# aconley/mbb_emcee

Hardware: AMD Instinct MI355X
Metric: walker-likelihood evals/sec (+ MCMC steps/sec), 250 walkers × 8 bands, 1/2/4/8 GPU (higher is better)
Workload: dtype f64; 1 GPU; cfg2/cfg3: 8 passbands (NQ 2209) with full response integration, thick+alpha, 250 walkers per GPU, device-resident stretch move; 1 step = 2 dependent half-steps; walkers_per_gpu=250, walkers=250, bands=8, nq=2209, sampler_form=form 7: one launch per <=4096 steps, preconditioning=50 ms of scratch-ensemble steps before the W warm-up steps (GPU clocks)

## Files before the change

### include/mbb_hip.h

```cpp
#ifndef MBB_HIP_H
#define MBB_HIP_H

#include <stddef.h>
#include <stdint.h>

#ifdef __cplusplus
extern "C" {
#endif

typedef struct mbb_ctx mbb_ctx;

enum mbb_error {
    MBB_OK = 0,
    MBB_ERR_HIP = -1,
    MBB_ERR_ARG = -2,
    MBB_ERR_STATE = -3,
    MBB_ERR_RCCL = -4
};

enum mbb_row_status {
    MBB_ROW_OK = 0,
    MBB_ROW_BELOW_LOWLIM = 1,
    MBB_ROW_BAD_ALPHA = 2,
    MBB_ROW_BAD_BETA = 3,
// ... 31 lines not shown
                            double *d_lnl, int32_t *d_status, double *d_model_flux);

int mbb_lnlike_repeat_device(mbb_ctx *ctx, const double *d_pars, int n, double *d_lnl,
                             int32_t *d_status, int reps);

int mbb_roof_probe(mbb_ctx *ctx, const double pars[5], int reps, double *seconds,
                   double *lane_slots, double *clock_mhz);

int mbb_sampler_create(mbb_ctx *ctx, int nwalkers, unsigned long long seed, void **sampler);
int mbb_sampler_destroy(mbb_ctx *ctx, void *sampler);
int mbb_sampler_reset(mbb_ctx *ctx, void *sampler);
int mbb_sampler_set_state(mbb_ctx *ctx, void *sampler, const double *pos, const double *lnprob);
int mbb_sampler_run(mbb_ctx *ctx, void *sampler, int nsteps, double stretch_a, double *chain,
                    double *lnprob, double *pos_out, double *lnprob_out, double *naccepted);
int mbb_sampler_advance_async(mbb_ctx *ctx, void *sampler, int nsteps, double stretch_a);
int mbb_sampler_advance_timed(mbb_ctx *ctx, void *sampler, int nsteps, double stretch_a, double *wall_s,
                              float *stream_ms);

#define MBB_SUMMARY_COLS 8
#define MBB_SUMMARY_MAX_PCT 8
enum mbb_summary_derived { MBB_SUM_PEAK = 1, MBB_SUM_LIR = 2, MBB_SUM_DUSTMASS = 4 };
enum mbb_summary_status {
    MBB_SUM_EMPTY = 1,
    MBB_SUM_HAS_NAN = 2,
    MBB_SUM_ABSENT = 4,
    MBB_SUM_ROW_SHIFT = 8
};
typedef struct mbb_summary_spec {
    int32_t npct;
    int32_t burn, thin;
// ... 71 lines not shown
```

### mbb_emcee_amd/_native.py

```python
import ctypes as C
import os

import numpy as np

_HERE = os.path.dirname(os.path.abspath(__file__))
LIB_PATH = os.path.join(_HERE, "libmbb_hip.so")

ROW_OK, ROW_BELOW_LOWLIM, ROW_BAD_ALPHA, ROW_BAD_BETA, ROW_NOCONV, ROW_NONFINITE = 0, 1, 2, 3, 6, 7

_dp = C.POINTER(C.c_double)
_ip = C.POINTER(C.c_int32)
_vp = C.c_void_p

SUMMARY_COLS, SUMMARY_MAX_PCT = 8, 8
SUM_PEAK, SUM_LIR, SUM_DUSTMASS = 1, 2, 4
SUM_EMPTY, SUM_HAS_NAN, SUM_ABSENT, SUM_ROW_SHIFT = 1, 2, 4, 8


class SummarySpec(C.Structure):
    _fields_ = [("npct", C.c_int32), ("burn", C.c_int32), ("thin", C.c_int32), ("derived", C.c_int32),
                ("peak_model", C.c_int32),
                ("has_lo", C.c_int32 * SUMMARY_COLS), ("has_hi", C.c_int32 * SUMMARY_COLS),
                ("pct", C.c_double * SUMMARY_MAX_PCT),
                ("lo", C.c_double * SUMMARY_COLS), ("hi", C.c_double * SUMMARY_COLS),
# ... 23 lines not shown
    "mbb_lnlike_call": (C.c_int, [_vp, C.c_int]),
    "mbb_boundary_generation": (_vp, [_vp]),
    "mbb_lnlike_batch_device": (C.c_int, [_vp, _vp, C.c_int, _vp, _vp, _vp]),
    "mbb_lnlike_repeat_device": (C.c_int, [_vp, _vp, C.c_int, _vp, _vp, C.c_int]),
    "mbb_roof_probe": (C.c_int, [_vp, _dp, C.c_int, _dp, _dp, _dp]),
    "mbb_sampler_create": (C.c_int, [_vp, C.c_int, C.c_ulonglong, C.POINTER(_vp)]),
    "mbb_sampler_destroy": (C.c_int, [_vp, _vp]),
    "mbb_sampler_reset": (C.c_int, [_vp, _vp]),
    "mbb_sampler_set_state": (C.c_int, [_vp, _vp, _dp, _dp]),
    "mbb_sampler_run": (C.c_int, [_vp, _vp, C.c_int, C.c_double, _dp, _dp, _dp, _dp, _dp]),
    "mbb_chain_summary": (C.c_int, [_vp, _dp, _dp, C.c_int, C.c_int, C.c_int, C.POINTER(SummarySpec),
                                    C.POINTER(SummaryOut)]),
    "mbb_sampler_run_summary": (C.c_int, [_vp, _vp, C.c_int, C.c_double, C.POINTER(SummarySpec),
                                          C.POINTER(SummaryOut), _dp, _dp, _dp, _dp, _dp]),
    "mbb_sampler_advance_async": (C.c_int, [_vp, _vp, C.c_int, C.c_double]),
    "mbb_sampler_advance_timed": (C.c_int, [_vp, _vp, C.c_int, C.c_double, C.POINTER(C.c_double), C.POINTER(C.c_float)]),
    "mbb_sed_prologue_batch": (C.c_int, [_vp, _dp, C.c_int, C.c_int, C.c_int, C.c_double,
                                         C.c_int, _dp, _ip]),
    "mbb_sed_eval_batch": (C.c_int, [_vp, _dp, C.c_int, C.c_int, C.c_int, C.c_double, _dp,
                                     C.c_int, _dp, _ip]),
    "mbb_sed_integrate_batch": (C.c_int, [_vp, _dp, C.c_int, C.c_int, C.c_int, C.c_double, C.c_double,
                                          C.c_double, _dp, _ip]),
    "mbb_fnu_eval": (C.c_int, [_vp, C.c_int, C.c_int, _dp, C.c_int] + [C.c_double] * 7 + [_dp]),
    "mbb_malloc": (C.c_int, [_vp, C.c_size_t, C.POINTER(_vp)]),
    "mbb_free": (C.c_int, [_vp, _vp]),
    "mbb_memcpy_h2d": (C.c_int, [_vp, _vp, _vp, C.c_size_t]),
    "mbb_memcpy_d2h": (C.c_int, [_vp, _vp, _vp, C.c_size_t]),
    "mbb_sync": (C.c_int, [_vp]),
    "mbb_stream": (_vp, [_vp]),
    "mbb_event_create": (C.c_int, [_vp, C.POINTER(_vp)]),
# ... 329 lines not shown
```

### mbb_emcee_amd/csrc/mbb_flow_index.h

```cpp
#pragma once
#if defined(__HIPCC__)
#define MBB_FLOW_HD __host__ __device__
#else
#define MBB_FLOW_HD
#endif

constexpr int kFlowSlots = 4;
constexpr int kFlowLag = 4;

MBB_FLOW_HD constexpr int flow_cnt(int h, int j) { return (j - h + 1) > 0 ? (j - h + 1) >> 1 : 0; }
MBB_FLOW_HD constexpr int flow_seq(int h, int m) { return m > 0 ? h + 2 * m - 1 : 0; }

constexpr int kFmSlots = 4;
constexpr int kFmMseq = kFmSlots;
constexpr int kFmLag = 4;
constexpr int kFmRing = 8;
constexpr int kFmNC = 3;
constexpr int kFmNB = 4;
```

### mbb_emcee_amd/csrc/mbb_flowa.hip.h

```cpp
#pragma once
#include "mbb_flowm.hip.h"


template <bool OPTHIN, bool NOALPHA, bool STAGE>
__global__ void __launch_bounds__(1024) k_flowa(const LikeArgs a_val)
{
    CLikeArgs *const ka = MBB_KERNARGS();
    extern __shared__ __align__(16) unsigned char smem_raw[];
    __shared__ __align__(16) double s_tab[kExp2N];
    __shared__ __align__(16) double s_pb[kPolyBDoubles];
    __shared__ __align__(16) double s_pc[OPTHIN ? 2 : kPolyCDoubles];
    const int tid = threadIdx.x, lane = tid & 63, wave = MBB_WAVE_ID(tid);
#define MBB_FA_COMMON() \
    const int W = a.wpb; \
    const int nun = a.nunit, npart = a.npart, nb = a.nb; \
    const int nC = (2 * W + 3) >> 2, nQ = 16 - nC; \
    WalkerK *wk0 = reinterpret_cast<WalkerK *>(smem_raw);                          \
    double *partial0 = reinterpret_cast<double *>(wk0 + kFaNB * W);               \
    double *rec0 = partial0 + kFaNB * (size_t)W * npart;                          \
    double *mflux = rec0 + kFaNB * (size_t)W * kFaRec;                            \
    double *own = mflux + (size_t)W * nb;                                         \
    double *s_flux = own + 2 * (size_t)W * 8; \
    double *s_ivar = s_flux + nb; \
    double *s_invcov = s_ivar + nb; \
    int2 *s_band = reinterpret_cast<int2 *>(s_invcov + (a.cov_in_lds ? (size_t)nb * nb : 0)); \
    int *ctl = reinterpret_cast<int *>(s_band + nb + 1);                          \
    const size_t tab_off = ((size_t)(reinterpret_cast<unsigned char *>(ctl + 48) - smem_raw) + 15) & ~(size_t)15; \
    double *s_nu = reinterpret_cast<double *>(smem_raw + tab_off); \
    double *s_lnnu = s_nu + (STAGE ? a.nchunk * 64 : 0); \
    double *s_wt = s_lnnu + (STAGE ? a.nchunk * 64 : 0); \
    const int wbase = (int)blockIdx.x * W; \
    const int Wl = min(W, a.n - wbase); \
    const FlowMView fv = flowm_view(a.spec, a.nw); \
    const unsigned long long serial32 = a.flow_serial << 32; \
    unsigned long long *const done_set = fv.done + (size_t)(a.spec_cfg & 1) * kFmRing * 16; \
    const long long spin_limit = flow_spin_limit(a.spec_cfg); \
    const int niter = a.persist; \
    int *const c_ready = ctl + 16, *const c_qdone = ctl + 32, *const c_edone = ctl + 4; \
    (void)nun; (void)nQ; (void)mflux; (void)own; (void)s_flux; (void)s_ivar; (void)s_invcov; (void)s_nu; (void)s_lnnu; (void)s_wt; \
    (void)Wl; (void)done_set; (void)spin_limit; (void)niter; (void)c_ready; (void)c_qdone; (void)c_edone; (void)partial0; (void)rec0

    {
        MBB_ROLE_ARGS();
        MBB_FA_COMMON();
        const int nt = (int)blockDim.x;
        if (tid < 48) ctl[tid] = 0;
        if (tid < 2 * W * 6) {
            const int hh = tid / (W * 6), l = (tid - hh * W * 6) / 6, e = tid % 6;
            if (l < Wl) {
                const int r = (hh ? a.c_count : 0) + wbase + l;
                const double v = a.pos6[(size_t)r * 6 + e];
                own[(size_t)(hh * W + l) * 8 + e] = v;
                fm_put(fv.row + (size_t)r * kFmWords + 2 * e, v, serial32);
            }
        }
        if (blockIdx.x == 0 && tid < kFmRing * 16)
            __hip_atomic_store(fv.done + (size_t)((a.spec_cfg & 1) ^ 1) * kFmRing * 16 + tid, 0ull, __ATOMIC_RELAXED, __HIP_MEMORY_SCOPE_AGENT);
        const double2 *gb = reinterpret_cast<const double2 *>(a.poly_b);
        const double2 *gc = reinterpret_cast<const double2 *>(a.poly_c);
        double2 *lb = reinterpret_cast<double2 *>(s_pb);
        double2 *lc = reinterpret_cast<double2 *>(s_pc);
        for (int i = tid; i < kExp2N; i += nt) s_tab[i] = kExp2Tab[i];
        for (int i = tid; i < kPolyBDoubles / 2; i += nt) lb[i] = gb[i];
        if (!OPTHIN)
            for (int i = tid; i < kPolyCDoubles / 2; i += nt) lc[i] = gc[i];
        for (int b = tid; b < nb; b += nt) { s_flux[b] = a.flux[b]; s_ivar[b] = a.ivar[b]; s_band[b] = a.band_rng[b]; }
        if (a.cov_in_lds)
            for (int i = tid; i < nb * nb; i += nt) s_invcov[i] = a.invcov[i];
        if (STAGE) {
            const int n2 = a.nchunk * 32;
            const double2 *g0 = reinterpret_cast<const double2 *>(a.nu), *g1 = reinterpret_cast<const double2 *>(a.lnnu),
                          *g2 = reinterpret_cast<const double2 *>(a.wt);
// ... 206 lines not shown
            const int row = sb + wbase + l;
            const bool c1 = cand && j > 0;
            const bool active = l < Wl && (cand == 0 || j > 0);
            double zz = 1.0, u3 = 0.5;
            int pj = 0;
            if (active) stretch_draw(row, a.step + (j >> 1), h, a.seed + 0x9E3779B97F4A7C15ull * (unsigned long long)(j >> 1),
                                     a.stretch_a, a.c_count, zz, pj, u3);
            const int prow = ob + pj;
            const int m1 = flow_cnt(h ^ 1, j), m0 = flow_cnt(h ^ 1, j - 1);
            if (j >= kFaNB) lds_wait(c_edone + bj, Wl * MBB_FA_TURN(j - kFaNB));
            const double *src = c1 ? fv.prop + (((size_t)prow * kFmSlots + (m1 % kFmSlots)) * 2) * kFmWords + 2 * (l16 < 5 ? l16 : 0)
                                   : fv.row + ((size_t)(m0 % kFmSlots) * a.nw + prow) * kFmWords + 2 * (l16 < 5 ? l16 : 0);
            const unsigned long long tag = serial32 | (unsigned long long)(c1 ? j : flow_seq(h ^ 1, m0));
            const bool want_e = active && l16 < 5, want_g = ci == 0 && lane == 5 && j >= kFmLag;
            const unsigned long long need_g = (unsigned long long)gridDim.x * (unsigned long long)nC * (unsigned long long)(((j - kFmLag) / kFmRing) + 1);
            const unsigned long long *gword = done_set + ((j - kFmLag) & (kFmRing - 1)) * 16;
            if (ci == 0) FA_EV(j, 8);
            double pv = 0.0;
            {
                bool ok = !(want_e || want_g);
                long long spins = 0;
                for (;;) {
                    if (want_e && !ok) ok = fm_get(src, tag, pv);
                    if (want_g && !ok) ok = __hip_atomic_load(gword, __ATOMIC_RELAXED, __HIP_MEMORY_SCOPE_AGENT) >= need_g;
                    if (__builtin_amdgcn_ballot_w64(!ok) == 0) break;
                    ++spins;
                    if (spins > spin_limit ||
                        ((spins & 255) == 8 && __hip_atomic_load(a.errflag, __ATOMIC_RELAXED, __HIP_MEMORY_SCOPE_AGENT) != 0)) {
                        atomicMax(a.errflag, 9);
                        break;
                    }
// ... 53 lines not shown
                    if (now && lane == pbase) __hip_atomic_store(c_ready + bj * 8 + l, MBB_FA_TURN(j), __ATOMIC_RELAXED, __HIP_MEMORY_SCOPE_WORKGROUP);
                    if (__builtin_amdgcn_ballot_w64(!handed) == 0) break;
                    ++spins;
                    if (spins > spin_limit ||
                        ((spins & 255) == 8 && __hip_atomic_load(a.errflag, __ATOMIC_RELAXED, __HIP_MEMORY_SCOPE_AGENT) != 0)) {
                        atomicMax(a.errflag, 9);
                        break;
                    }
                    __builtin_amdgcn_s_sleep(1);
                    if (watch2 && !handed) v2 = __hip_atomic_load(w2, __ATOMIC_RELAXED, __HIP_MEMORY_SCOPE_AGENT);
                }
            }
            if (ci == 0) FA_EV(j, 11);
            MBB_FM_ORDER();
            if (ci == 0) FA_EV(j, 12);
            if (lane == 0) __hip_atomic_fetch_add(done_set + (j & (kFmRing - 1)) * 16, 1ull, __ATOMIC_RELAXED, __HIP_MEMORY_SCOPE_AGENT);
        }
    }
#undef MBB_FA_COMMON
#undef MBB_FA_TURN
#undef FA_EV
}
```

### mbb_emcee_amd/csrc/mbb_flowm.hip.h

```cpp
#pragma once
#include "mbb_kernels.hip.h"

__device__ __forceinline__ long long flow_spin_limit(int spec_cfg)
{
    const int v = (spec_cfg >> 24) & 0x3f;
    return v == 63 ? 0ll : 1ll << (v ? v : 22);
}

constexpr int kFmReady = 0;
constexpr int kFmQDone = 4;
constexpr int kFmEDone = 8;
constexpr int kFmPen = 16;
constexpr int kFmStaged = 12;
constexpr int kFmLooks = 8;
constexpr int kFmPrioChain = 3, kFmPrioCtor = 2, kFmPrioWait = 1;

__device__ __forceinline__ int fm_loop_lane(int l)
{
    asm volatile("" : "+v"(l));
    return l;
}
__device__ __forceinline__ void fm_put(double *pair, double v, unsigned long long tag)
{
    typedef unsigned int u32x4 __attribute__((ext_vector_type(4)));
// ... 40 lines not shown
    double *s_ivar = s_flux + nb; \
    double *s_invcov = s_ivar + nb; \
    int2 *s_band = reinterpret_cast<int2 *>(s_invcov + (a.cov_in_lds ? (size_t)nb * nb : 0)); \
    double *cscr = reinterpret_cast<double *>(s_band + nb + 1); \
    int *ctl0 = reinterpret_cast<int *>(cscr + kFmNC * 64); \
    const size_t unit_off = ((size_t)(reinterpret_cast<unsigned char *>(ctl0 + 32 * NP) - smem_raw) + 15) & ~(size_t)15; \
    int4 *s_unit = reinterpret_cast<int4 *>(smem_raw + unit_off);     \
    int *s_tail = reinterpret_cast<int *>(s_unit + nun);               \
    const size_t tab_off = unit_off + (size_t)kFmUnitBytes * nun; \
    double *s_nu = reinterpret_cast<double *>(smem_raw + tab_off); \
    double *s_lnnu = s_nu + (STAGE ? a.nchunk * 64 : 0); \
    double *s_wt = s_lnnu + (STAGE ? a.nchunk * 64 : 0); \
    const long long spin_limit = flow_spin_limit(a.spec_cfg); \
    const FlowMView fv = flowm_view(a.spec, a.nw); \
    const unsigned long long serial32 = a.flow_serial << 32; \
    unsigned long long *const done_set = fv.done + (size_t)(a.spec_cfg & 1) * kFmRing * 16; \
    const int niter = a.persist;
#define MBB_FM_PAIRS_LOOP _Pragma("clang loop unroll(disable)")
#define MBB_FM_PAIR(vp) \
    const int w = wbase + (vp); \
    if constexpr (NP > 1) { if (w >= a.n) continue; }       \
    WalkerK *const wk = wk0 + (vp) * kFmNB; \
    double *const partial = partial0 + (size_t)(vp) * kFmNB * npart; \
    double *const prop = prop0 + (vp) * kFmNB * kFmProp; \
    int *const ctl = ctl0 + 32 * (vp); \
    (void)wk; (void)partial; (void)prop; (void)ctl
#define MBB_FM_ORDER() do { __builtin_amdgcn_fence(__ATOMIC_ACQ_REL, "wavefront"); __builtin_amdgcn_wave_barrier(); } while (0)
#define MBB_FM_WAITS() \
    auto dec_ok = [&](unsigned long long v, unsigned long long need) {    \
        return (v >> 32) == (serial32 >> 32) && ((v & 0xffffffffull) >> 1) >= need; \
    }; \
// ... 33 lines not shown
    const int tid = threadIdx.x, lane = tid & 63, wave = MBB_WAVE_ID(tid);
    const int nwave = blockDim.x >> 6, nq = nwave - kFmNC - 2;
    const bool spread = nwave == 16;
    const int role = spread ? (wave == 3 ? 1 : wave == 7 ? 2 : wave == 14 ? 3 : wave == 11 ? 1 + kFmNC : wave == 15 ? 2 + kFmNC : 0)
                            : (wave < nq ? 0 : 1 + wave - nq);
    const int qi = spread ? wave - (wave >> 2) : wave;
    {
        MBB_ROLE_ARGS();
        MBB_FM_COMMON();
        if (tid < 32 * NP) ctl0[tid] = 0;
        if (cand == 0 && tid < 12 * NP && wbase + tid / 12 < a.n) {
            const int t12 = tid % 12;
            const int r = (t12 < 6 ? 0 : a.c_count) + wbase + tid / 12, e = t12 < 6 ? t12 : t12 - 6;
            fm_put(fv.row + (size_t)r * kFmWords + 2 * e, a.pos6[(size_t)r * 6 + e], serial32);
        }
        if (blockIdx.x == 0 && tid < kFmRing * 16)
            __hip_atomic_store(fv.done + (size_t)((a.spec_cfg & 1) ^ 1) * kFmRing * 16 + tid, 0ull, __ATOMIC_RELAXED, __HIP_MEMORY_SCOPE_AGENT);
        (void)done_set; (void)niter; (void)spin_limit;
    }
    __syncthreads();
#ifdef MBB_STAMPS
    if (tid == 0 && a.stamps) a.stamps[(1u << 20) + 4096 + blockIdx.x] = __builtin_amdgcn_s_memrealtime();
    unsigned long long t_acc[8] = {0, 0, 0, 0, 0, 0, 0, 0};
    unsigned long long t_last = __builtin_amdgcn_s_memtime();
#define FM_T(kk) do { const unsigned long long t_now = __builtin_amdgcn_s_memtime(); t_acc[kk] += t_now - t_last; t_last = t_now; } while (0)
#define FM_TD(kk, dep) do { asm volatile("" ::"v"(dep)); FM_T(kk); } while (0)
#define FM_TOUT() do { if (lane == 0 && a.stamps) for (int kk = 0; kk < 8; ++kk) a.stamps[((size_t)blockIdx.x * 16 + wave) * 8 + kk] = t_acc[kk]; } while (0)
    if (lane == 0 && a.stamps) {
        unsigned hwid, xcc;
        asm volatile("s_getreg_b32 %0, hwreg(HW_REG_HW_ID)" : "=s"(hwid));
        asm volatile("s_getreg_b32 %0, hwreg(HW_REG_XCC_ID)" : "=s"(xcc));
        a.stamps[(1u << 20) + blockIdx.x * 16 + wave] = ((unsigned long long)xcc << 32) | hwid;
// ... 145 lines not shown
        MBB_FM_PAIRS_LOOP
        for (int vp = 0; vp < NP; ++vp) {
            MBB_FM_PAIR(vp);
            const int b = it & (kFmNB - 1);
            const int L_step = a.step + (it >> 1), L_half = it & 1;
            const unsigned long long L_seed = a.seed + 0x9E3779B97F4A7C15ull * (unsigned long long)(it >> 1);
            const int row = (L_half ? a.c_count : 0) + w, c_begin = L_half ? 0 : a.c_count;
            double zz, u3;
            int pj;
            stretch_draw(row, L_step, L_half, L_seed, a.stretch_a, a.c_count, zz, pj, u3);
            const int prow = c_begin + pj;
            const int m_par = flow_cnt(L_half ^ 1, it), m_s = flow_cnt(L_half, it);
            const unsigned long long need_p = (unsigned long long)flow_seq(L_half ^ 1, m_par);
            const double *lnp_p = fv.row + ((size_t)(m_s % kFmSlots) * a.nw + row) * kFmWords + 10;
            const unsigned long long tag_s = serial32 | (unsigned long long)flow_seq(L_half, m_s);
            const unsigned long long need_g = 2ull * (unsigned long long)a.n * (unsigned long long)(((it - kFmLag) / kFmRing) + 1);
            const unsigned long long *word = lane == 22 ? fv.mseq + (size_t)prow * kFmMseq + (m_par % kFmSlots)
                                                        : done_set + ((it - kFmLag) & (kFmRing - 1)) * 16;
            const bool watch = (lane == 22 && need_p > 0) || (lane == 23 && it >= kFmLag);
            const WalkerK *wkb = wk + b;
            const double *pr = prop + b * kFmProp;
            int st = ROW_SKIP;
            double cbb = 0.0, pen_u = 0.0, pen_g = 0.0, lnz4 = 0.0, lnu = 0.0, acc = 0.0;
            double q[5] = {0.0, 0.0, 0.0, 0.0, 0.0}, old5[5] = {0.0, 0.0, 0.0, 0.0, 0.0};
            bool have_rec = false;
            auto record = [&]() {
                st = wkb->status;
                cbb = wkb->cq; pen_u = pr[7]; pen_g = pr[8];
#pragma unroll
                for (int i = 0; i < 5; ++i) { q[i] = pr[i]; old5[i] = pr[9 + i]; }
                lnz4 = pr[5]; lnu = pr[6];
                have_rec = true;
            };
            auto sums = [&]() {
// ... 40 lines not shown
            };
            const int q_need = nq * ((it / kFmNB) + 1);
            FM_EV(it, 9);
#ifdef MBB_STAMPS
            unsigned long long t_ok = 0;
#endif
            unsigned long long pv = 0;
            double lnp = 0.0;
            bool ok = !(watch || lane == 21), have_sums = false;
            long long spins = 0;
            __builtin_amdgcn_s_setprio(kFmPrioWait);
            for (;;) {
                double lv;
                unsigned long long lchk, wv;
                const bool ask_l = lane == 21 && !ok, ask_w = watch && !ok;
                if (ask_l) {
                    lv = ld_dev(lnp_p);
                    lchk = __hip_atomic_load(reinterpret_cast<const unsigned long long *>(lnp_p) + 1, __ATOMIC_RELAXED, __HIP_MEMORY_SCOPE_AGENT);
                }
                if (ask_w) wv = __hip_atomic_load(word, __ATOMIC_RELAXED, __HIP_MEMORY_SCOPE_AGENT);
#pragma nounroll
                for (int look = 0; !have_sums; ++look) {
                    if (!have_rec && __hip_atomic_load(ctl + kFmPen + b, __ATOMIC_RELAXED, __HIP_MEMORY_SCOPE_WORKGROUP) >= it + 1) {
                        MBB_FM_ORDER();
                        record();
                    }
                    if (__hip_atomic_load(ctl + kFmQDone + b, __ATOMIC_RELAXED, __HIP_MEMORY_SCOPE_WORKGROUP) >= q_need) {
                        MBB_FM_ORDER();
                        FM_EV(it, 4);
                        sums();
                        have_sums = true;
                        break;
                    }
                    if (look >= kFmLooks) break;
                    __builtin_amdgcn_s_sleep(1);
                }
                if (ask_l) asm volatile("" : "+v"(lv), "+v"(lchk));
                if (ask_w) asm volatile("" : "+v"(wv));
                if (ask_l) { lnp = lv; ok = (lchk ^ (unsigned long long)__double_as_longlong(lv)) == tag_s; }
                if (ask_w) { pv = wv; ok = lane == 22 ? dec_ok(pv, need_p) : pv >= need_g; }
#ifdef MBB_STAMPS
                if ((ask_l || ask_w) && ok) t_ok = __builtin_amdgcn_s_memrealtime();
#endif
                if (__builtin_amdgcn_ballot_w64(!ok) == 0) break;
                ++spins;
                if (spins > spin_limit ||
                    ((spins & 255) == 8 && __hip_atomic_load(a.errflag, __ATOMIC_RELAXED, __HIP_MEMORY_SCOPE_AGENT) != 0)) {
                    atomicMax(a.errflag, 9);
                    break;
                }
                __builtin_amdgcn_s_sleep(1);
            }
            __builtin_amdgcn_s_setprio(kFmPrioChain);
            const int flag = (need_p > 0 && (fm_lane_lo<22>(pv) & 1u)) ? 1 : 0;
            const bool mine = flag == cand;
            const double lnp_cur = fm_lane<21>(lnp);
            FM_TD(0, lnp_cur);
            FM_EV(it, 5);
            FM_EVV(it, 7, prow);
#ifdef MBB_STAMPS
            { const unsigned long long t21 = __shfl(t_ok, 21), t22 = __shfl(t_ok, 22), t23 = __shfl(t_ok, 23);
              FM_EVV(it, 10, t21); FM_EVV(it, 11, t22); FM_EVV(it, 12, t23); }
#endif
            if (!have_sums) {
                lds_wait(ctl + kFmQDone + b, q_need);
                FM_T(1);
                FM_EV(it, 4);
                sums();
            }
            FM_TD(2, acc);
            {
                double r;
                if (st == ROW_BELOW_LOWLIM) r = -__builtin_inf();
                else if (st != ROW_OK) r = __builtin_nan("");
                else {
                    r = fma(-0.5, acc, pen_u);
// ... 10 lines not shown
                                           __HIP_MEMORY_SCOPE_AGENT);
                    const double lnp_new = accept ? r : lnp_cur;
                    double ve = lnp_new;
#pragma unroll
                    for (int i = 0; i < 5; ++i) ve = ((lane & 7) == i) ? (accept ? q[i] : old5[i]) : ve;
                    if (lane < 6)
                        fm_put(fv.row + ((size_t)(m_new % kFmSlots) * a.nw + row) * kFmWords + 2 * lane, ve,
                               serial32 | (unsigned long long)(it + 1));
                    __builtin_amdgcn_s_setprio(kFmPrioWait);
                    if (lane < 6) { if (it + 2 >= niter) a.pos6[(size_t)row * 6 + lane] = ve; }
                    else if (lane >= 8 && lane < 14 && a.chain6)
                        a.chain6[((size_t)it * a.n + w) * 6 + (lane - 8)] = ve;
                    if (lane == 0 && accept) atomicAdd(a.nacc + (size_t)L_half * a.n + w, 1u);
                }
                __builtin_amdgcn_s_setprio(kFmPrioWait);
                if (lane == 0) __hip_atomic_fetch_add(done_set + (it & (kFmRing - 1)) * 16, 1ull, __ATOMIC_RELAXED, __HIP_MEMORY_SCOPE_AGENT);
            }
            FM_T(3);
        }
        FM_TOUT();
        return;
    }

    {
        MBB_ROLE_ARGS();
        MBB_FM_COMMON();
        MBB_FM_WAITS();
        MBB_PIN(a.c_count); MBB_PIN(a.step); MBB_PIN(a.seed); MBB_PIN(a.stretch_a); MBB_PIN(a.nw); MBB_PIN(a.errflag); MBB_PIN(a.zpow);
        MBB_PIN(a.lowlim[0]); MBB_PIN(a.lowlim[1]); MBB_PIN(a.lowlim[2]); MBB_PIN(a.lowlim[3]); MBB_PIN(a.lowlim[4]);
        MBB_PIN(a.nunorm); MBB_PIN(a.lnunorm); MBB_PIN(a.has_uplim); MBB_PIN(a.has_gprior);
        const int cb = role - 1;
// ... 197 lines not shown
```

### mbb_emcee_amd/csrc/mbb_hip.hip

```cpp
#include <hip/hip_runtime.h>
#include <dlfcn.h>
#include <math.h>
#include <stdint.h>
#include <stdio.h>
#include <stdlib.h>
#include <string.h>
#include <time.h>

#include <algorithm>
#include <functional>
#include <string>
#include <type_traits>
#include <atomic>
#include <chrono>
#include <mutex>
#include <thread>
#include <vector>

#include "../../include/mbb_hip.h"
#include "mbb_device.hip.h"
#include "mbb_kernels.hip.h"
#include "mbb_summary.hip.h"

#define MBB_FLOW_EXT(OT, NA)                                                    \
// ... 1147 lines not shown
    if (rc) return rc;
    mbb_sampler_state *s = (mbb_sampler_state *)sp;
    if (!s) return MBB_OK;
    HIPCHK(hipStreamSynchronize(c->stream));
    if (s->pos6_owned) free_dev(s->d_pos6);
    else if (c->x.users > 0) --c->x.users;
    free_dev(s->d_nacc); free_dev(s->d_err); free_dev(s->d_chain6); free_dev(s->d_chain_out); free_dev(s->d_spec);
    if (s->h_chain) (void)hipHostFree(s->h_chain);
    free_dev(s->d_bak);
    delete s;
    return MBB_OK;
}

static int sampler_check_pending(mbb_ctx *c, mbb_sampler_state *s);

extern "C" int mbb_sampler_reset(mbb_ctx *c, void *sp)
{
    int rc = use(c);
    if (rc) return rc;
    mbb_sampler_state *s = (mbb_sampler_state *)sp;
    if (!s) return fail(MBB_ERR_ARG, "null sampler");
    (void)sampler_check_pending(c, s);
    HIPCHK(hipStreamSynchronize(c->stream));
    HIPCHK(hipMemset(s->d_nacc, 0, (size_t)s->rows() * sizeof(unsigned int)));
    HIPCHK(hipMemset(s->d_err, 0, sizeof(int)));
    return MBB_OK;
}

extern "C" int mbb_sampler_set_state(mbb_ctx *c, void *sp, const double *pos, const double *lnprob)
{
// ... 271 lines not shown
    if (rp.resting) --c->flow_rest;
    if (rp.form >= 7) {
        const size_t R = (size_t)s->rows();
        if (!s->d_spec) {
            HIPCHK(hipMalloc((void **)&s->d_spec, spec_words(R) * sizeof(double)));
            HIPCHK(hipMemsetAsync(s->d_spec, 0, spec_words(R) * sizeof(double), c->stream));
        }
        if (backup) {
            if (!s->d_bak) HIPCHK(hipMalloc((void **)&s->d_bak, R * 6 * sizeof(double) + R * sizeof(unsigned int)));
            HIPCHK(hipMemcpyAsync(s->d_bak, s->d_pos6, R * 6 * sizeof(double), hipMemcpyDeviceToDevice, c->stream));
            HIPCHK(hipMemcpyAsync(s->d_bak + R * 6, s->d_nacc, R * sizeof(unsigned int), hipMemcpyDeviceToDevice, c->stream));
        }
        s->backup_kept = backup;
        if (s->spec_form != 7 && s->spec_form != 9) {
            const FlowMView fvh = flowm_view(s->d_spec, (int)R);
            HIPCHK(hipMemsetAsync(fvh.done, 0, 2 * kFmRing * 16 * sizeof(unsigned long long), c->stream));
            s->flowm_parity = 0;
        }
        s->spec_form = rp.form;
    }
    const bool carried = tev && rp.form >= 7 && nsteps <= 4096;
    if (tev && !carried) HIPCHK(hipEventRecord(tev[0], c->stream));
    if (rp.p.xchg) {
        XchgArgs xa;
        memset(&xa, 0, sizeof xa);
        for (int r = 0; r < c->x.n; ++r) { xa.xpos[r] = c->x.pos6(r); xa.xflag[r] = c->x.flags(r); }
        xa.xcount = c->x.count(); xa.xn = c->x.n; xa.xrank = c->x.rank;
        xa.xseq0 = c->x.seq; xa.xspin_max = c->x.spin_max;
        HIPCHK(hipMemcpyAsync(c->x.d_args, &xa, sizeof xa, hipMemcpyHostToDevice, c->stream));
    }
    SamplerLaunch sl;
// ... 973 lines not shown
```

### mbb_emcee_amd/csrc/mbb_host_tables.cpp

```cpp
#include "mbb_host_tables.h"

#include <math.h>

#include <algorithm>
#include <functional>

namespace mbbh {

int build_band_layout(const double *freq, const double *weight, const int32_t *offsets, int nb,
                      int seg_chunks, bool pack_tails, BandLayout &L, const char **err)
{
    static const char *msgs[] = {"", "bad band tables", "offsets[0] must be 0", "empty band",
                                 "non-positive frequency"};
    auto bad = [&](int code) { if (err) *err = msgs[-code]; return code; };
    if (!freq || !weight || !offsets || nb <= 0) return bad(-1);
    if (offsets[0] != 0) return bad(-2);
    const int segc = seg_chunks > 0 ? seg_chunks : 4;
    for (int b = 0; b < nb; ++b) {
        if (offsets[b + 1] - offsets[b] <= 0) return bad(-3);
        for (int i = offsets[b]; i < offsets[b + 1]; ++i)
            if (!(freq[i] > 0.0) || !isfinite(freq[i])) return bad(-4);
    }
    L = BandLayout();
    std::vector<double> &nu = L.nu, &lnnu = L.lnnu, &wt = L.wt;
// ... 255 lines not shown
#include "mbb_flow_index.h"
extern "C" int mbbh_flow_index(int h, int j, int m, int *cnt, int *seq, int *slots, int *lag)
{
    *cnt = flow_cnt(h, j);
    *seq = flow_seq(h, m);
    *slots = kFlowSlots;
    *lag = kFlowLag;
    return 0;
}

extern "C" int mbbh_flowm_consts(int *slots, int *lag, int *ring, int *nc, int *nb)
{
    *slots = kFmSlots; *lag = kFmLag; *ring = kFmRing; *nc = kFmNC; *nb = kFmNB;
    return 0;
}
```

### mbb_emcee_amd/csrc/mbb_kernels.hip.h

```cpp
#pragma once
#include <hip/hip_runtime.h>
#include <stdint.h>

#include "mbb_device.hip.h"
#include "mbb_flow_index.h"
#include "mbb_lds_plans.hip.h"

using namespace mbbd;

constexpr int kPolyBDoubles = (mbbm::kPolyBMax * 8 + 1) * mbbm::kPolyStride;
constexpr int kPolyCDoubles = (mbbm::kPolyCMax * 8 + 1) * mbbm::kPolyStride;

struct XchgArgs {
    double *xpos[16];
    unsigned long long *xflag[16];
    unsigned int *xcount;
    int xn, xrank;
    unsigned long long xseq0;
    long long xspin_max;
};

struct LikeArgs {
    const double *nu;
    const double *lnnu;
// ... 49 lines not shown
        };
    };
};
#ifndef MBB_WC_ROW
#define MBB_WC_ROW true
#endif
constexpr int kPreWords = 16;
static_assert(sizeof(mbbd::WalkerK) == 13 * sizeof(double), "a walker's record is 13 words");
#ifndef MBB_SRV_STRIDE
#define MBB_SRV_STRIDE 8
#endif
constexpr int kSrvStride = MBB_SRV_STRIDE;
#ifndef MBB_STAMPS
static_assert(sizeof(LikeArgs) == 480, "the argument block: every launch of every variant pays for its size");
#endif
constexpr int kFlowRecN = 22, kFlowRec = 48;
struct FlowView {
    double *rec, *st;
    unsigned long long *seq, *done, *mseq, *pub, *startf, *endf;
};
__host__ __device__ constexpr size_t spec_words(size_t nw)
{
    return nw * ((size_t)kFlowSlots * 2 * kFlowRec + kFlowSlots * 8 + 1 + kFlowSlots) + 8 * 16 + 16 * 8 + 32;
}
__host__ __device__ __forceinline__ FlowView flow_view(double *spec, int nw)
{
    FlowView v;
    v.rec = spec;
    v.st = spec + (size_t)nw * kFlowSlots * 2 * kFlowRec;
    v.seq = reinterpret_cast<unsigned long long *>(v.st + (size_t)nw * kFlowSlots * 8);
    v.done = v.seq + nw;
    v.mseq = v.done + 8 * 16;
    v.pub = v.mseq + (size_t)nw * kFlowSlots;
    v.startf = v.pub + 16 * 8;
    v.endf = v.startf + 16;
    return v;
}
struct FlowX {
    double *base[16];
// ... 888 lines not shown
    const int r = rh / per, loc = rh - r * per;
    const size_t nl = (size_t)nsrc * per;
    const size_t w = (size_t)src * per + loc;
    const double *q = chain6 + ((((size_t)r * nsteps + t) * 2 + h) * nl + w) * 6;
    double *c = out + (size_t)i * 5;
#pragma unroll
    for (int k = 0; k < 5; ++k) c[k] = q[k];
    out[(size_t)R * nsteps * 5 + i] = q[5];
    (void)shards;
}

struct FlowMView {
    double *prop, *row;
    unsigned long long *mseq, *done;
};
constexpr int kFmWords = 16;
__host__ __device__ constexpr size_t flowm_words(size_t nw)
{
    return ((nw * ((size_t)kFmSlots * 2 * kFmWords + kFmSlots * kFmWords + kFmMseq) + 31) & ~(size_t)31) + 2 * kFmRing * 16;
}
static_assert(flowm_words(1000) <= spec_words(1000) && flowm_words(2) <= spec_words(2), "form 7 lives in the allocation of forms 5/6");
__host__ __device__ __forceinline__ FlowMView flowm_view(double *spec, int nw)
{
    FlowMView v;
    v.prop = spec;
    v.row = spec + (size_t)nw * kFmSlots * 2 * kFmWords;
    v.mseq = reinterpret_cast<unsigned long long *>(v.row + (size_t)nw * kFmSlots * kFmWords);
    v.done = reinterpret_cast<unsigned long long *>(spec) + (flowm_words((size_t)nw) - 2 * kFmRing * 16);
    return v;
}
static __global__ void k_flow_post(const FlowX *fx, int nw, int which, unsigned long long run, const int *errflag)
{
    const int pr = threadIdx.x;
    if (pr >= fx->n) return;
    __builtin_amdgcn_fence(__ATOMIC_RELEASE, "");
    const FlowView v = flow_view(fx->base[pr], nw);
    const unsigned long long bad = (which && errflag && *errflag != 0) ? (1ull << 63) : 0ull;
    __hip_atomic_store((which ? v.endf : v.startf) + fx->rank, run | bad, __ATOMIC_RELAXED, __HIP_MEMORY_SCOPE_SYSTEM);
}

static __global__ void k_flow_wait_end(const unsigned long long *endf, int xn, int xrank, unsigned long long run,
                                       long long spin_max, int *errflag)
{
// ... 219 lines not shown
```

### mbb_emcee_amd/device_sampler.py

```python
import ctypes as C

import numpy as np

from . import _native
from .ensemble import integrated_time

__all__ = ["DeviceEnsembleSampler"]


class DeviceEnsembleSampler(object):

    def __init__(self, nwalkers, dim, lnpostfn, a=2.0, threads=1, seed=None, **unused):
        if dim != 5:
            raise ValueError("the modified blackbody model has 5 parameters")
        if nwalkers % 2 != 0:
            raise ValueError("The number of walkers must be even.")
        if nwalkers < 2 * dim:
            raise ValueError("The number of walkers needs to be more than twice the "
                             "dimension of your parameter space.")
        if not hasattr(lnpostfn, "_sync_device"):
            raise TypeError("DeviceEnsembleSampler needs a mbb_emcee_amd.likelihood")
        self.k, self.dim, self.a = int(nwalkers), 5, float(a)
        self.lnprobfn = lnpostfn
        self.seed = int(np.random.SeedSequence(seed).generate_state(1, dtype=np.uint64)[0]) \
# ... 215 lines not shown
                        self._chain, self._lnprob = kept_c, kept_l
                    self.iterations = it_prev + done
                    self.naccepted = acc_made if j == k - 1 else acc_before + moved[..., j]
                    yield steps[..., j, :], lnps[..., j], self.seed
        finally:
            self.iterations, self.naccepted = it_prev + made, acc_made
            if storechain:
                self._chain, self._lnprob = big_c[..., :n_prev + made, :], big_l[..., :n_prev + made]
            else:
                self._chain, self._lnprob = kept_c, kept_l

    def advance_async(self, N):
        ctx, h = self._handle()
        _native._check(ctx.lib.mbb_sampler_advance_async(ctx.h, h, int(N), self.a))

    def advance_timed(self, N):
        ctx, h = self._handle()
        wall, ms = C.c_double(), C.c_float()
        _native._check(ctx.lib.mbb_sampler_advance_timed(ctx.h, h, int(N), self.a, C.byref(wall), C.byref(ms)))
        return wall.value, ms.value

    def __del__(self):
        try:
            if self._h is not None and self._ctx is not None and self._ctx.h:
                self._ctx.lib.mbb_sampler_destroy(self._ctx.h, self._h)
        except Exception:
            pass
```

Measured before the change: 50.99 million evals/s.

## Shard the form-7 grid-wide done counters across four cache lines

Measured after the change: 51.73 million evals/s (median of 6 runs). +1.4%, better.

```diff
diff --git a/include/mbb_hip.h b/include/mbb_hip.h
--- a/include/mbb_hip.h
+++ b/include/mbb_hip.h
@@ -69,6 +69,8 @@
 int mbb_sampler_run(mbb_ctx *ctx, void *sampler, int nsteps, double stretch_a, double *chain,
                     double *lnprob, double *pos_out, double *lnprob_out, double *naccepted);
 int mbb_sampler_advance_async(mbb_ctx *ctx, void *sampler, int nsteps, double stretch_a);
+int mbb_sampler_flow_counters(mbb_ctx *ctx, void *sampler, unsigned long long *counters, int cap, int store, int *ring,
+                              int *shards, int *next_set);
 int mbb_sampler_advance_timed(mbb_ctx *ctx, void *sampler, int nsteps, double stretch_a, double *wall_s,
                               float *stream_ms);
 
diff --git a/mbb_emcee_amd/_native.py b/mbb_emcee_amd/_native.py
--- a/mbb_emcee_amd/_native.py
+++ b/mbb_emcee_amd/_native.py
@@ -61,6 +61,8 @@
     "mbb_sampler_run_summary": (C.c_int, [_vp, _vp, C.c_int, C.c_double, C.POINTER(SummarySpec),
                                           C.POINTER(SummaryOut), _dp, _dp, _dp, _dp, _dp]),
     "mbb_sampler_advance_async": (C.c_int, [_vp, _vp, C.c_int, C.c_double]),
+    "mbb_sampler_flow_counters": (C.c_int, [_vp, _vp, C.POINTER(C.c_ulonglong), C.c_int, C.c_int, C.POINTER(C.c_int),
+                                            C.POINTER(C.c_int), C.POINTER(C.c_int)]),
     "mbb_sampler_advance_timed": (C.c_int, [_vp, _vp, C.c_int, C.c_double, C.POINTER(C.c_double), C.POINTER(C.c_float)]),
     "mbb_sed_prologue_batch": (C.c_int, [_vp, _dp, C.c_int, C.c_int, C.c_int, C.c_double,
                                          C.c_int, _dp, _ip]),
diff --git a/mbb_emcee_amd/csrc/mbb_flow_index.h b/mbb_emcee_amd/csrc/mbb_flow_index.h
--- a/mbb_emcee_amd/csrc/mbb_flow_index.h
+++ b/mbb_emcee_amd/csrc/mbb_flow_index.h
@@ -1,4 +1,5 @@
 #pragma once
+#include <stddef.h>
 #if defined(__HIPCC__)
 #define MBB_FLOW_HD __host__ __device__
 #else
@@ -15,5 +16,23 @@
 constexpr int kFmMseq = kFmSlots;
 constexpr int kFmLag = 4;
 constexpr int kFmRing = 8;
+constexpr int kFmShards = 4;
+constexpr int kFmDoneLine = 16;
+constexpr int kFmDoneWords = 2 * kFmRing * kFmShards * kFmDoneLine;
+static_assert((kFmShards & (kFmShards - 1)) == 0 && kFmShards >= 1 && kFmShards <= 32, "shards: a power of two, one reader lane each");
+MBB_FLOW_HD constexpr int fm_shard(int wg) { return wg & (kFmShards - 1); }
+MBB_FLOW_HD constexpr int fm_shard_wgs(int grid, int s) { return grid > s ? (grid - s + kFmShards - 1) / kFmShards : 0; }
+MBB_FLOW_HD constexpr int fm_done_word(int set, int slot, int s) { return ((set * kFmRing + slot) * kFmShards + s) * kFmDoneLine; }
+constexpr int kFmWords = 16;
+MBB_FLOW_HD constexpr size_t flowm_mseq_end(size_t nw) { return nw * ((size_t)kFmSlots * 2 * kFmWords + kFmSlots * kFmWords + kFmMseq); }
+MBB_FLOW_HD constexpr size_t flowm_words(size_t nw)
+{
+    return ((flowm_mseq_end(nw) + 31) & ~(size_t)31) + kFmDoneWords;
+}
+constexpr int kFlowRecN = 22, kFlowRec = 48;
+MBB_FLOW_HD constexpr size_t spec_words(size_t nw)
+{
+    return nw * ((size_t)kFlowSlots * 2 * kFlowRec + kFlowSlots * 8 + 1 + kFlowSlots) + 8 * 16 + 16 * 8 + 32 + kFmDoneWords;
+}
 constexpr int kFmNC = 3;
 constexpr int kFmNB = 4;
diff --git a/mbb_emcee_amd/csrc/mbb_flowa.hip.h b/mbb_emcee_amd/csrc/mbb_flowa.hip.h
--- a/mbb_emcee_amd/csrc/mbb_flowa.hip.h
+++ b/mbb_emcee_amd/csrc/mbb_flowa.hip.h
@@ -33,7 +33,7 @@
     const int Wl = min(W, a.n - wbase); \
     const FlowMView fv = flowm_view(a.spec, a.nw); \
     const unsigned long long serial32 = a.flow_serial << 32; \
-    unsigned long long *const done_set = fv.done + (size_t)(a.spec_cfg & 1) * kFmRing * 16; \
+    unsigned long long *const done_set = fv.done + fm_done_word(a.spec_cfg & 1, 0, 0);       \
     const long long spin_limit = flow_spin_limit(a.spec_cfg); \
     const int niter = a.persist; \
     int *const c_ready = ctl + 16, *const c_qdone = ctl + 32, *const c_edone = ctl + 4; \
@@ -54,8 +54,9 @@
                 fm_put(fv.row + (size_t)r * kFmWords + 2 * e, v, serial32);
             }
         }
-        if (blockIdx.x == 0 && tid < kFmRing * 16)
-            __hip_atomic_store(fv.done + (size_t)((a.spec_cfg & 1) ^ 1) * kFmRing * 16 + tid, 0ull, __ATOMIC_RELAXED, __HIP_MEMORY_SCOPE_AGENT);
+        if (blockIdx.x == 0 && tid < kFmRing * kFmShards)
+            __hip_atomic_store(fv.done + fm_done_word((a.spec_cfg & 1) ^ 1, tid / kFmShards, tid % kFmShards), 0ull, __ATOMIC_RELAXED,
+                               __HIP_MEMORY_SCOPE_AGENT);
         const double2 *gb = reinterpret_cast<const double2 *>(a.poly_b);
         const double2 *gc = reinterpret_cast<const double2 *>(a.poly_c);
         double2 *lb = reinterpret_cast<double2 *>(s_pb);
@@ -292,7 +293,7 @@
             const unsigned long long tag = serial32 | (unsigned long long)(c1 ? j : flow_seq(h ^ 1, m0));
             const bool want_e = active && l16 < 5, want_g = ci == 0 && lane == 5 && j >= kFmLag;
             const unsigned long long need_g = (unsigned long long)gridDim.x * (unsigned long long)nC * (unsigned long long)(((j - kFmLag) / kFmRing) + 1);
-            const unsigned long long *gword = done_set + ((j - kFmLag) & (kFmRing - 1)) * 16;
+            const unsigned long long *gword = done_set + fm_done_word(0, (j - kFmLag) & (kFmRing - 1), 0);
             if (ci == 0) FA_EV(j, 8);
             double pv = 0.0;
             {
@@ -376,7 +377,7 @@
             if (ci == 0) FA_EV(j, 11);
             MBB_FM_ORDER();
             if (ci == 0) FA_EV(j, 12);
-            if (lane == 0) __hip_atomic_fetch_add(done_set + (j & (kFmRing - 1)) * 16, 1ull, __ATOMIC_RELAXED, __HIP_MEMORY_SCOPE_AGENT);
+            if (lane == 0) __hip_atomic_fetch_add(done_set + fm_done_word(0, j & (kFmRing - 1), 0), 1ull, __ATOMIC_RELAXED, __HIP_MEMORY_SCOPE_AGENT);
         }
     }
 #undef MBB_FA_COMMON
diff --git a/mbb_emcee_amd/csrc/mbb_flowm.hip.h b/mbb_emcee_amd/csrc/mbb_flowm.hip.h
--- a/mbb_emcee_amd/csrc/mbb_flowm.hip.h
+++ b/mbb_emcee_amd/csrc/mbb_flowm.hip.h
@@ -78,7 +78,7 @@
     const long long spin_limit = flow_spin_limit(a.spec_cfg); \
     const FlowMView fv = flowm_view(a.spec, a.nw); \
     const unsigned long long serial32 = a.flow_serial << 32; \
-    unsigned long long *const done_set = fv.done + (size_t)(a.spec_cfg & 1) * kFmRing * 16; \
+    unsigned long long *const done_set = fv.done + fm_done_word(a.spec_cfg & 1, 0, 0); \
     const int niter = a.persist;
 #define MBB_FM_PAIRS_LOOP _Pragma("clang loop unroll(disable)")
 #define MBB_FM_PAIR(vp) \
@@ -142,8 +142,9 @@
             const int r = (t12 < 6 ? 0 : a.c_count) + wbase + tid / 12, e = t12 < 6 ? t12 : t12 - 6;
             fm_put(fv.row + (size_t)r * kFmWords + 2 * e, a.pos6[(size_t)r * 6 + e], serial32);
         }
-        if (blockIdx.x == 0 && tid < kFmRing * 16)
-            __hip_atomic_store(fv.done + (size_t)((a.spec_cfg & 1) ^ 1) * kFmRing * 16 + tid, 0ull, __ATOMIC_RELAXED, __HIP_MEMORY_SCOPE_AGENT);
+        if (blockIdx.x == 0 && tid < kFmRing * kFmShards)
+            __hip_atomic_store(fv.done + fm_done_word((a.spec_cfg & 1) ^ 1, tid / kFmShards, tid % kFmShards), 0ull, __ATOMIC_RELAXED,
+                               __HIP_MEMORY_SCOPE_AGENT);
         (void)done_set; (void)niter; (void)spin_limit;
     }
     __syncthreads();
@@ -319,10 +320,11 @@
             const unsigned long long need_p = (unsigned long long)flow_seq(L_half ^ 1, m_par);
             const double *lnp_p = fv.row + ((size_t)(m_s % kFmSlots) * a.nw + row) * kFmWords + 10;
             const unsigned long long tag_s = serial32 | (unsigned long long)flow_seq(L_half, m_s);
-            const unsigned long long need_g = 2ull * (unsigned long long)a.n * (unsigned long long)(((it - kFmLag) / kFmRing) + 1);
+            const int gsh = (lane - 23) & (kFmShards - 1);
+            const unsigned long long need_g = (unsigned long long)fm_shard_wgs(2 * a.n, gsh) * (unsigned long long)(((it - kFmLag) / kFmRing) + 1);
             const unsigned long long *word = lane == 22 ? fv.mseq + (size_t)prow * kFmMseq + (m_par % kFmSlots)
-                                                        : done_set + ((it - kFmLag) & (kFmRing - 1)) * 16;
-            const bool watch = (lane == 22 && need_p > 0) || (lane == 23 && it >= kFmLag);
+                                                        : done_set + fm_done_word(0, (it - kFmLag) & (kFmRing - 1), gsh);
+            const bool watch = (lane == 22 && need_p > 0) || (lane >= 23 && lane < 23 + kFmShards && it >= kFmLag && need_g > 0);
             const WalkerK *wkb = wk + b;
             const double *pr = prop + b * kFmProp;
             int st = ROW_SKIP;
@@ -393,6 +395,9 @@
                 double lv;
                 unsigned long long lchk, wv;
                 const bool ask_l = lane == 21 && !ok, ask_w = watch && !ok;
+#ifdef MBB_STAMPS
+                const unsigned long long t_ask = __builtin_amdgcn_s_memrealtime();
+#endif
                 if (ask_l) {
                     lv = ld_dev(lnp_p);
                     lchk = __hip_atomic_load(reinterpret_cast<const unsigned long long *>(lnp_p) + 1, __ATOMIC_RELAXED, __HIP_MEMORY_SCOPE_AGENT);
@@ -419,7 +424,11 @@
                 if (ask_l) { lnp = lv; ok = (lchk ^ (unsigned long long)__double_as_longlong(lv)) == tag_s; }
                 if (ask_w) { pv = wv; ok = lane == 22 ? dec_ok(pv, need_p) : pv >= need_g; }
 #ifdef MBB_STAMPS
-                if ((ask_l || ask_w) && ok) t_ok = __builtin_amdgcn_s_memrealtime();
+                if ((ask_l || ask_w) && ok) {
+                    t_ok = __builtin_amdgcn_s_memrealtime();
+                    const unsigned long long dt = t_ok - t_ask;
+                    t_ok = (t_ok & ((1ull << 52) - 1)) | ((dt > 4095ull ? 4095ull : dt) << 52);
+                }
 #endif
                 if (__builtin_amdgcn_ballot_w64(!ok) == 0) break;
                 ++spins;
@@ -438,7 +447,11 @@
             FM_EV(it, 5);
             FM_EVV(it, 7, prow);
 #ifdef MBB_STAMPS
-            { const unsigned long long t21 = __shfl(t_ok, 21), t22 = __shfl(t_ok, 22), t23 = __shfl(t_ok, 23);
+            { unsigned long long t21 = __shfl(t_ok, 21), t22 = __shfl(t_ok, 22), t23 = __shfl(t_ok, 23);
+              for (int sh = 1; sh < kFmShards; ++sh) {
+                  const unsigned long long ts = __shfl(t_ok, 23 + sh);
+                  if ((ts & ((1ull << 52) - 1)) > (t23 & ((1ull << 52) - 1))) t23 = ts;
+              }
               FM_EVV(it, 10, t21); FM_EVV(it, 11, t22); FM_EVV(it, 12, t23); }
 #endif
             if (!have_sums) {
@@ -479,7 +492,9 @@
                     if (lane == 0 && accept) atomicAdd(a.nacc + (size_t)L_half * a.n + w, 1u);
                 }
                 __builtin_amdgcn_s_setprio(kFmPrioWait);
-                if (lane == 0) __hip_atomic_fetch_add(done_set + (it & (kFmRing - 1)) * 16, 1ull, __ATOMIC_RELAXED, __HIP_MEMORY_SCOPE_AGENT);
+                if (lane == 0)
+                    __hip_atomic_fetch_add(done_set + fm_done_word(0, it & (kFmRing - 1), fm_shard((int)blockIdx.x)), 1ull, __ATOMIC_RELAXED,
+                                           __HIP_MEMORY_SCOPE_AGENT);
             }
             FM_T(3);
         }
diff --git a/mbb_emcee_amd/csrc/mbb_hip.hip b/mbb_emcee_amd/csrc/mbb_hip.hip
--- a/mbb_emcee_amd/csrc/mbb_hip.hip
+++ b/mbb_emcee_amd/csrc/mbb_hip.hip
@@ -1185,6 +1185,32 @@
 
 static int sampler_check_pending(mbb_ctx *c, mbb_sampler_state *s);
 
+extern "C" int mbb_sampler_flow_counters(mbb_ctx *c, void *sp, unsigned long long *counters, int cap, int store, int *ring,
+                                         int *shards, int *next_set)
+{
+    int rc = use(c);
+    if (rc) return rc;
+    mbb_sampler_state *s = (mbb_sampler_state *)sp;
+    const int n = 2 * kFmRing * kFmShards;
+    if (!s || !counters || !ring || !shards || !next_set || cap < n) return fail(MBB_ERR_ARG, "bad arguments");
+    if (!s->d_spec || (s->spec_form != 7 && s->spec_form != 9))
+        return fail(MBB_ERR_STATE, "the sampler holds no state of a one-launch run (forms 7, 9)");
+    HIPCHK(hipStreamSynchronize(c->stream));
+    const FlowMView fv = flowm_view(s->d_spec, s->rows());
+    std::vector<unsigned long long> w(kFmDoneWords);
+    HIPCHK(hipMemcpy(w.data(), fv.done, w.size() * sizeof(unsigned long long), hipMemcpyDeviceToHost));
+    for (int set = 0; set < 2; ++set)
+        for (int slot = 0; slot < kFmRing; ++slot)
+            for (int sh = 0; sh < kFmShards; ++sh) {
+                unsigned long long &word = w[fm_done_word(set, slot, sh)], &val = counters[(set * kFmRing + slot) * kFmShards + sh];
+                if (store) word = val;
+                else val = word;
+            }
+    if (store) HIPCHK(hipMemcpy(fv.done, w.data(), w.size() * sizeof(unsigned long long), hipMemcpyHostToDevice));
+    *ring = kFmRing; *shards = kFmShards; *next_set = s->flowm_parity;
+    return MBB_OK;
+}
+
 extern "C" int mbb_sampler_reset(mbb_ctx *c, void *sp)
 {
     int rc = use(c);
@@ -1486,7 +1512,7 @@
         s->backup_kept = backup;
         if (s->spec_form != 7 && s->spec_form != 9) {
             const FlowMView fvh = flowm_view(s->d_spec, (int)R);
-            HIPCHK(hipMemsetAsync(fvh.done, 0, 2 * kFmRing * 16 * sizeof(unsigned long long), c->stream));
+            HIPCHK(hipMemsetAsync(fvh.done, 0, kFmDoneWords * sizeof(unsigned long long), c->stream));
             s->flowm_parity = 0;
         }
         s->spec_form = rp.form;
diff --git a/mbb_emcee_amd/csrc/mbb_host_tables.cpp b/mbb_emcee_amd/csrc/mbb_host_tables.cpp
--- a/mbb_emcee_amd/csrc/mbb_host_tables.cpp
+++ b/mbb_emcee_amd/csrc/mbb_host_tables.cpp
@@ -293,3 +293,16 @@
     *slots = kFmSlots; *lag = kFmLag; *ring = kFmRing; *nc = kFmNC; *nb = kFmNB;
     return 0;
 }
+
+extern "C" int mbbh_flowm_guard(int grid, int wg, int set, int slot, int shard, int nw, int *shards, int *wg_shard,
+                                int *shard_wgs, long long *word, long long *mseq_end, long long *words, long long *alloc_words)
+{
+    *shards = kFmShards;
+    *wg_shard = fm_shard(wg);
+    *shard_wgs = fm_shard_wgs(grid, shard);
+    *words = (long long)flowm_words((size_t)nw);
+    *word = *words - kFmDoneWords + fm_done_word(set, slot, shard);
+    *mseq_end = (long long)flowm_mseq_end((size_t)nw);
+    *alloc_words = (long long)spec_words((size_t)nw);
+    return 0;
+}
diff --git a/mbb_emcee_amd/csrc/mbb_kernels.hip.h b/mbb_emcee_amd/csrc/mbb_kernels.hip.h
--- a/mbb_emcee_amd/csrc/mbb_kernels.hip.h
+++ b/mbb_emcee_amd/csrc/mbb_kernels.hip.h
@@ -87,15 +87,10 @@
 #ifndef MBB_STAMPS
 static_assert(sizeof(LikeArgs) == 480, "the argument block: every launch of every variant pays for its size");
 #endif
-constexpr int kFlowRecN = 22, kFlowRec = 48;
 struct FlowView {
     double *rec, *st;
     unsigned long long *seq, *done, *mseq, *pub, *startf, *endf;
 };
-__host__ __device__ constexpr size_t spec_words(size_t nw)
-{
-    return nw * ((size_t)kFlowSlots * 2 * kFlowRec + kFlowSlots * 8 + 1 + kFlowSlots) + 8 * 16 + 16 * 8 + 32;
-}
 __host__ __device__ __forceinline__ FlowView flow_view(double *spec, int nw)
 {
     FlowView v;
@@ -1014,11 +1009,6 @@
     double *prop, *row;
     unsigned long long *mseq, *done;
 };
-constexpr int kFmWords = 16;
-__host__ __device__ constexpr size_t flowm_words(size_t nw)
-{
-    return ((nw * ((size_t)kFmSlots * 2 * kFmWords + kFmSlots * kFmWords + kFmMseq) + 31) & ~(size_t)31) + 2 * kFmRing * 16;
-}
 static_assert(flowm_words(1000) <= spec_words(1000) && flowm_words(2) <= spec_words(2), "form 7 lives in the allocation of forms 5/6");
 __host__ __device__ __forceinline__ FlowMView flowm_view(double *spec, int nw)
 {
@@ -1026,7 +1016,7 @@
     v.prop = spec;
     v.row = spec + (size_t)nw * kFmSlots * 2 * kFmWords;
     v.mseq = reinterpret_cast<unsigned long long *>(v.row + (size_t)nw * kFmSlots * kFmWords);
-    v.done = reinterpret_cast<unsigned long long *>(spec) + (flowm_words((size_t)nw) - 2 * kFmRing * 16);
+    v.done = reinterpret_cast<unsigned long long *>(spec) + (flowm_words((size_t)nw) - kFmDoneWords);
     return v;
 }
 static __global__ void k_flow_post(const FlowX *fx, int nw, int which, unsigned long long run, const int *errflag)
diff --git a/mbb_emcee_amd/device_sampler.py b/mbb_emcee_amd/device_sampler.py
--- a/mbb_emcee_amd/device_sampler.py
+++ b/mbb_emcee_amd/device_sampler.py
@@ -253,6 +253,19 @@
         ctx, h = self._handle()
         _native._check(ctx.lib.mbb_sampler_advance_async(ctx.h, h, int(N), self.a))
 
+    def flow_counters(self, store=None):
+        ctx, h = self._handle()
+        buf = (C.c_ulonglong * 256)()
+        ring, shards, nxt = C.c_int(), C.c_int(), C.c_int()
+        if store is not None:
+            flat = np.asarray(store, dtype=np.uint64).reshape(-1)
+            for i, v in enumerate(flat):
+                buf[i] = int(v)
+            _native._check(ctx.lib.mbb_sampler_flow_counters(ctx.h, h, buf, 256, 1, C.byref(ring), C.byref(shards), C.byref(nxt)))
+        _native._check(ctx.lib.mbb_sampler_flow_counters(ctx.h, h, buf, 256, 0, C.byref(ring), C.byref(shards), C.byref(nxt)))
+        n = 2 * ring.value * shards.value
+        return np.array(buf[:n], dtype=np.uint64).reshape(2, ring.value, shards.value), nxt.value
+
     def advance_timed(self, N):
         ctx, h = self._handle()
         wall, ms = C.c_double(), C.c_float()
```
